# ckallidonis/mugiq

Hardware: AMD Instinct MI355X
Metric: loop_trace_sites_per_sec (higher is better)
Workload: dtype f64; 1 GPU; 32x32x32x32 fp64 N_ev=200 ultra-local 16-gamma loop (order FLOAT2); n_ev=200, partition=independent site blocks, one per rank

## Files before the change

### mugiq_amd/csrc/prolong.hip

```cpp
#include "mg_common.h"

#include <algorithm>
#include <vector>

namespace mugiq {

template <typename F, typename A> struct ProlongArgs {
  const Cplx<F> *V;
  int64_t Vpo;
  int Vstride;
  int NV;
  int X[4], Xc[4], bs[4];
  int spinBs;
  int volumeCB;
  const void *const *coarse;
  int64_t Cpo;
  int Cstride;
  const void *const *fine;
  int Fstride;
  int64_t Fpo;
  int nVec;
  const A *inv_sigma;
  Cplx<A> *loop;
};

template <typename F, typename A, int ORDER, bool WRITE, bool CONTRACT, bool STAGED>
__global__ __launch_bounds__(kPrTile *kPrGroups) void prolong_kernel(ProlongArgs<F, A> a) {
  extern __shared__ __align__(16) unsigned char smem[];
  Cplx<F> *Vt = reinterpret_cast<Cplx<F> *>(smem);
  const int tilesPerParity = (a.volumeCB + kPrTile - 1) / kPrTile;
  const int pty = blockIdx.x / tilesPerParity;
  const int x0 = (blockIdx.x - pty * tilesPerParity) * kPrTile;
  const int t = threadIdx.x, site = t & (kPrTile - 1), g = t / kPrTile;
  const int x_cb = x0 + site;
  const bool valid = x_cb < a.volumeCB;

  if constexpr (STAGED) {
    const int nPl = 12 * a.NV;
    for (int k = g; k < nPl; k += kPrGroups)
      Vt[k * kPrTile + site] = valid ? a.V[pty * a.Vpo + (int64_t)k * a.Vstride + x_cb] : Cplx<F>{F(0), F(0)};
    __syncthreads();
  }
  const Cplx<F> *Vg = a.V + pty * a.Vpo + (valid ? x_cb : a.volumeCB - 1);

  int c[4] = {0, 0, 0, 0};
  if (valid) get_coords(c, x_cb, a.X, pty);
  int cc[4];
#pragma unroll
  for (int d = 0; d < 4; d++) cc[d] = c[d] / a.bs[d];
  const int cpar = (cc[0] + cc[1] + cc[2] + cc[3]) & 1;
  const int64_t coff = (int64_t)cpar * a.Cpo + (lex_index(cc, a.Xc) >> 1);

  A diag[4] = {A(0), A(0), A(0), A(0)};
  Cplx<A> up[6];
#pragma unroll
  for (int i = 0; i < 6; i++) up[i] = Cplx<A>{A(0), A(0)};

  for (int nb = 0; nb < a.nVec; nb += 2 * kPrGroups) {
    const int n0 = nb + 2 * g, n1 = n0 + 1;
    if (n0 >= a.nVec) continue;
    const bool has1 = n1 < a.nVec;
    const Cplx<F> *c0 = static_cast<const Cplx<F> *>(a.coarse[n0]) + coff;
    const Cplx<F> *c1 = static_cast<const Cplx<F> *>(a.coarse[has1 ? n1 : n0]) + coff;
    Cplx<A> o0[12], o1[12];
#pragma unroll
    for (int k = 0; k < 12; k++) o0[k] = o1[k] = Cplx<A>{A(0), A(0)};
    typedef F vec2 __attribute__((ext_vector_type(2)));
    Cplx<F> sv0[12], sv1[12], sv2[12];
    vec2 sp0[4], sp1[4], sp2[4];
#define MUGIQ_PR_LOAD(sv, sp, jexpr)                                                                                   \
  {                                                                                                                    \
    const int j_ = (jexpr) < a.NV ? (jexpr) : a.NV - 1;                                                                \
    _Pragma("unroll") for (int chi = 0; chi < 2; chi++) {                                                              \
      sp[chi] = *as_global(reinterpret_cast<const vec2 *>(c0 + (int64_t)(chi * a.NV + j_) * a.Cstride));               \
      sp[2 + chi] = *as_global(reinterpret_cast<const vec2 *>(c1 + (int64_t)(chi * a.NV + j_) * a.Cstride));           \
    }                                                                                                                  \
    _Pragma("unroll") for (int sc = 0; sc < 12; sc++) {                                                                \
      if constexpr (STAGED) sv[sc] = Vt[(sc * a.NV + j_) * kPrTile + site];                                            \
      else sv[sc] = Vg[(int64_t)(sc * a.NV + j_) * a.Vstride];                                                         \
    }                                                                                                                  \
  }
#define MUGIQ_PR_COMPUTE(sv, sp)                                                                                       \
  {                                                                                                                    \
    const Cplx<A> p0[2] = {Cplx<A>{(A)sp[0].x, (A)sp[0].y}, Cplx<A>{(A)sp[1].x, (A)sp[1].y}};                          \
    const Cplx<A> p1[2] = {Cplx<A>{(A)sp[2].x, (A)sp[2].y}, Cplx<A>{(A)sp[3].x, (A)sp[3].y}};                          \
    _Pragma("unroll") for (int sc = 0; sc < 12; sc++) {                                                                \
      const Cplx<A> v{(A)sv[sc].re, (A)sv[sc].im};                                                                     \
      const int chi = (sc / 3) / 2;               \
      cmadd(o0[sc], v, p0[chi]);                                                                                       \
      cmadd(o1[sc], v, p1[chi]);                                                                                       \
    }                                                                                                                  \
  }
    if constexpr (CONTRACT) {
      for (int j = 0; j < a.NV; j++) {
        MUGIQ_PR_LOAD(sv0, sp0, j)
        MUGIQ_PR_COMPUTE(sv0, sp0)
      }
    } else {
      MUGIQ_PR_LOAD(sv0, sp0, 0)
      MUGIQ_PR_LOAD(sv1, sp1, 1)
      for (int j = 0; j < a.NV; j += 3) {
        MUGIQ_PR_LOAD(sv2, sp2, j + 2)
        MUGIQ_PR_COMPUTE(sv0, sp0)
        MUGIQ_PR_LOAD(sv0, sp0, j + 3)
        if (j + 1 < a.NV) MUGIQ_PR_COMPUTE(sv1, sp1)
        MUGIQ_PR_LOAD(sv1, sp1, j + 4)
        if (j + 2 < a.NV) MUGIQ_PR_COMPUTE(sv2, sp2)
      }
    }
#undef MUGIQ_PR_LOAD
#undef MUGIQ_PR_COMPUTE
    if constexpr (WRITE) {
      if (valid) {
        Cplx<F> w[12];
#pragma unroll
        for (int k = 0; k < 12; k++) w[k] = Cplx<F>{(F)o0[k].re, (F)o0[k].im};
        SpinorView<F, ORDER>{const_cast<F *>(static_cast<const F *>(a.fine[n0])), a.Fstride, a.Fpo}.store(w, pty, x_cb);
        if (has1) {
#pragma unroll
          for (int k = 0; k < 12; k++) w[k] = Cplx<F>{(F)o1[k].re, (F)o1[k].im};
          SpinorView<F, ORDER>{const_cast<F *>(static_cast<const F *>(a.fine[n1])), a.Fstride, a.Fpo}.store(w, pty, x_cb);
        }
      }
    }
    if constexpr (CONTRACT) {
      accumulate_herm(diag, up, o0, a.inv_sigma[n0]);
      if (has1) accumulate_herm(diag, up, o1, a.inv_sigma[n1]);
    }
  }

  if constexpr (CONTRACT) {
    __syncthreads();
    A *red = reinterpret_cast<A *>(smem);
#pragma unroll
    for (int i = 0; i < 4; i++) red[(i * kPrGroups + g) * kPrTile + site] = diag[i];
#pragma unroll
    for (int i = 0; i < 6; i++) {
      red[((4 + 2 * i) * kPrGroups + g) * kPrTile + site] = up[i].re;
      red[((5 + 2 * i) * kPrGroups + g) * kPrTile + site] = up[i].im;
    }
    __syncthreads();
    if (g == 0 && valid) {
      A sum[16];
#pragma unroll
      for (int i = 0; i < 16; i++) {
        A s = A(0);
        for (int gg = 0; gg < kPrGroups; gg++) s += red[(i * kPrGroups + gg) * kPrTile + site];
        sum[i] = s;
      }
      Cplx<A> acc[16];
      int p = 0;
#pragma unroll
      for (int be = 0; be < 4; be++) {
        acc[be * 4 + be] = Cplx<A>{sum[be], A(0)};
#pragma unroll
        for (int al = be + 1; al < 4; al++) {
          acc[be * 4 + al] = Cplx<A>{sum[4 + 2 * p], sum[5 + 2 * p]};
          acc[al * 4 + be] = Cplx<A>{sum[4 + 2 * p], -sum[5 + 2 * p]};
          p++;
        }
      }
      trace_and_store(a.loop, acc, 2 * a.volumeCB, x_cb + pty * a.volumeCB);
    }
  }
}

int validate_transfer(const MugiqHipTransfer *T, const MugiqHipCoarseField *c0, const char *who) {
  MUGIQ_REQUIRE(T && T->V, "%s: transfer / null vectors are NULL", who);
  MUGIQ_REQUIRE(T->precision == 4 || T->precision == 8, "%s: transfer precision %d", who, T->precision);
  MUGIQ_REQUIRE(T->nVec >= 1 && T->nVec <= 64, "%s: n_vec = %d must be in [1, 64]", who, T->nVec);
  MUGIQ_REQUIRE(T->spinBlockSize == 2, "%s: spin_block_size = %d (the reference's drivers use 2, tests/loop.cpp:569)", who, T->spinBlockSize);
  long long vol = 1, volc = 1;
  for (int d = 0; d < 4; d++) {
    MUGIQ_REQUIRE(T->X[d] > 0 && (T->X[d] & 1) == 0, "%s: fine X[%d] = %d must be positive and even", who, d, T->X[d]);
    MUGIQ_REQUIRE(T->geoBlockSize[d] >= 1 && T->X[d] % T->geoBlockSize[d] == 0, "%s: geo_block_size[%d] = %d does not divide X = %d", who, d, T->geoBlockSize[d], T->X[d]);
    const int xc = T->X[d] / T->geoBlockSize[d];
    MUGIQ_REQUIRE((xc & 1) == 0, "%s: coarse extent %d in dim %d must be even (even-odd coarse field)", who, xc, d);
    MUGIQ_REQUIRE(c0->X[d] == xc, "%s: coarse field X[%d] = %d, expected %d", who, d, c0->X[d], xc);
    vol *= T->X[d];
    volc *= xc;
  }
  MUGIQ_REQUIRE(T->stride >= vol / 2 && T->parity_offset >= (int64_t)12 * T->nVec * T->stride, "%s: V stride / parity_offset too small", who);
  MUGIQ_REQUIRE(c0->data && c0->precision == T->precision && c0->nSpin == 2 && c0->nColor == T->nVec, "%s: coarse field must have precision %d, nSpin 2, nColor %d", who, T->precision, T->nVec);
  MUGIQ_REQUIRE(c0->volumeCB == volc / 2 && c0->stride >= c0->volumeCB && c0->parity_offset >= (int64_t)2 * T->nVec * c0->stride, "%s: coarse field geometry mismatch", who);
  return MUGIQ_HIP_SUCCESS;
}

template <typename Args> static void set_lattices(Args &a, const TransferGeom &g) {
  for (int d = 0; d < 4; d++) a.X[d] = g.X[d], a.Xc[d] = g.Xc[d], a.bs[d] = g.bs[d];
}
template <typename Args> static void set_geometry(Args &a, const TransferGeom &g) {
  set_lattices(a, g);
  a.volumeCB = g.volumeCB, a.volumeCBc = g.volumeCBc, a.aggVol = g.aggVol;
}

template <typename F, typename A, int ORDER, bool WRITE, bool CONTRACT, typename Form>
static int launch_prolong(const Form &form, bool staged, const MugiqHipTransfer *T, const MugiqHipCoarseField *coarse, const MugiqHipSpinorField *fine,
                          const double *sigma, void *loop_d, int nVec, hipStream_t stream) {
  const size_t pb = sizeof(void *) * (size_t)nVec;
  std::vector<unsigned char> host(2 * pb + sizeof(A) * (size_t)nVec);
  const void **hc = reinterpret_cast<const void **>(host.data());
  const void **hf = reinterpret_cast<const void **>(host.data() + pb);
  A *hs = reinterpret_cast<A *>(host.data() + 2 * pb);
  for (int n = 0; n < nVec; n++) {
    hc[n] = coarse[n].data;
    hf[n] = WRITE ? fine[n].data : nullptr;
    hs[n] = CONTRACT ? static_cast<A>(1.0 / static_cast<F>(sigma[n])) : A(0);
  }
  void *dev = nullptr;
  int st = upload_table(&dev, host.data(), host.size(), stream);
  if (st) return st;
  ProlongArgs<F, A> a;
  a.V = static_cast<const Cplx<F> *>(T->V);
  a.Vpo = T->parity_offset;
  a.Vstride = T->stride;
  a.NV = T->nVec;
  set_lattices(a, form.geom);
  a.spinBs = T->spinBlockSize;
  a.volumeCB = form.geom.volumeCB;
  a.coarse = reinterpret_cast<const void *const *>(dev);
  a.Cpo = coarse[0].parity_offset;
  a.Cstride = coarse[0].stride;
  a.fine = reinterpret_cast<const void *const *>(static_cast<unsigned char *>(dev) + pb);
  a.Fstride = WRITE ? fine[0].stride : 0;
  a.Fpo = WRITE ? fine[0].parity_offset : 0;
  a.nVec = nVec;
  a.inv_sigma = reinterpret_cast<const A *>(static_cast<unsigned char *>(dev) + 2 * pb);
  a.loop = static_cast<Cplx<A> *>(loop_d);
  if constexpr (sizeof(F) == 8)
    if (!staged) return launch_with_lds(prolong_kernel<F, A, ORDER, WRITE, CONTRACT, false>, form.workgroups, form.threads, form.ldsBytes, stream, a);
  return launch_with_lds(prolong_kernel<F, A, ORDER, WRITE, CONTRACT, true>, form.workgroups, form.threads, form.ldsBytes, stream, a);
}


constexpr int kPcEvecs = 8;
template <typename F> struct ProlongCoarseArgs {
  const Cplx<F> *V;
  int64_t Vpo;
  int Vstride, NV, NCf;
  int X[4], Xc[4], bs[4];
  int volumeCB;
  const void *const *in;
  int64_t Ipo, Opo;
  int Istride, Ostride, nVec;
};

template <typename F> __global__ __launch_bounds__(128) void prolong_coarse_kernel(ProlongCoarseArgs<F> a) {
  const int tid = blockIdx.x * blockDim.x + threadIdx.x;
  if (tid >= 2 * a.volumeCB) return;
  const int pty = tid / a.volumeCB, x_cb = tid - pty * a.volumeCB;
  const int k = blockIdx.y, s = k / a.NCf;
  const int n0 = blockIdx.z * kPcEvecs;
  int c[4], cc[4];
  get_coords(c, x_cb, a.X, pty);
#pragma unroll
  for (int d = 0; d < 4; d++) cc[d] = c[d] / a.bs[d];
  const int cpar = (cc[0] + cc[1] + cc[2] + cc[3]) & 1;
  const int64_t coff = (int64_t)cpar * a.Ipo + (lex_index(cc, a.Xc) >> 1);
  const Cplx<F> *inp[kPcEvecs];
#pragma unroll
  for (int i = 0; i < kPcEvecs; i++) {
    const int n = n0 + i < a.nVec ? n0 + i : a.nVec - 1;
    inp[i] = static_cast<const Cplx<F> *>(as_constant(a.in)[n]) + coff + (int64_t)(s * a.NV) * a.Istride;
  }
  Cplx<F> acc[kPcEvecs];
#pragma unroll
  for (int i = 0; i < kPcEvecs; i++) acc[i] = Cplx<F>{F(0), F(0)};
  const Cplx<F> *vp = a.V + (int64_t)pty * a.Vpo + (int64_t)k * a.NV * a.Vstride + x_cb;
  for (int j = 0; j < a.NV; j++) {
    const Cplx<F> v = vp[(int64_t)j * a.Vstride];
#pragma unroll
    for (int i = 0; i < kPcEvecs; i++) {
      typedef F vec2 __attribute__((ext_vector_type(2)));
      const vec2 u = *as_global(reinterpret_cast<const vec2 *>(inp[i] + (int64_t)j * a.Istride));
      cmadd(acc[i], v, Cplx<F>{u.x, u.y});
    }
  }
#pragma unroll
  for (int i = 0; i < kPcEvecs; i++)
    if (n0 + i < a.nVec) {
      Cplx<F> *o = static_cast<Cplx<F> *>(const_cast<void *>(as_constant(a.in)[a.nVec + n0 + i]));
      o[(int64_t)pty * a.Opo + (int64_t)k * a.Ostride + x_cb] = acc[i];
    }
}

template <typename F>
static int launch_prolong_coarse(const MugiqHipCoarseField *out, const MugiqHipCoarseField *in, int nVec, const MugiqHipTransfer *T,
                                 hipStream_t stream) {
  std::vector<const void *> host(2 * (size_t)nVec);
  for (int n = 0; n < nVec; n++) {
    host[n] = in[n].data;
    host[nVec + n] = out[n].data;
  }
  void *dev = nullptr;
  int st = upload_table(&dev, host.data(), host.size() * sizeof(void *), stream);
  if (st) return st;
  ProlongCoarseArgs<F> a;
  a.V = static_cast<const Cplx<F> *>(T->V);
  a.Vpo = T->parity_offset;
  a.Vstride = T->stride;
  a.NV = T->nVec;
  a.NCf = out[0].nColor;
  set_lattices(a, transfer_geom(*T));
  a.volumeCB = out[0].volumeCB;
  a.in = reinterpret_cast<const void *const *>(dev);
  a.Ipo = in[0].parity_offset;
  a.Istride = in[0].stride;
  a.Opo = out[0].parity_offset;
  a.Ostride = out[0].stride;
  a.nVec = nVec;
  const dim3 grid((2 * a.volumeCB + 127) / 128, 2 * a.NCf, (nVec + kPcEvecs - 1) / kPcEvecs);
  hipLaunchKernelGGL((prolong_coarse_kernel<F>), grid, dim3(128), 0, stream, a);
  MUGIQ_CHECK_HIP(hipGetLastError());
  return MUGIQ_HIP_SUCCESS;
}

template <typename F, typename A> struct CoarseOuterArgs {
  const void *const *coarse;
  const A *inv_sigma;
  int nVec, NV, volumeCBc, Cstride;
  int64_t Cpo;
  Cplx<A> *C;
};

constexpr int kCoEvecs = 8;
constexpr int kCoMaxNC = 64;

template <typename F, typename A, int B> __global__ __launch_bounds__(256) void coarse_outer_kernel(CoarseOuterArgs<F, A> a) {
  __shared__ Cplx<A> ph[kCoEvecs][kCoMaxNC], phs[kCoEvecs][kCoMaxNC];
  const int NC = 2 * a.NV;
  const int site = xcd_contiguous_block(blockIdx.x, gridDim.x);
  const int pty = site / a.volumeCBc, x_cb = site - pty * a.volumeCBc;
  const int r0 = (threadIdx.x >> 4) * B, c0 = (threadIdx.x & 15) * B;
  Cplx<A> acc[B][B];
#pragma unroll
  for (int i = 0; i < B; i++)
#pragma unroll
    for (int j = 0; j < B; j++) acc[i][j] = Cplx<A>{A(0), A(0)};
  for (int n0 = 0; n0 < a.nVec; n0 += kCoEvecs) {
    __syncthreads();
    for (int idx = threadIdx.x; idx < kCoEvecs * kCoMaxNC; idx += 256) {
      const int nn = idx / kCoMaxNC, comp = idx - nn * kCoMaxNC, n = n0 + nn;
      Cplx<A> v{A(0), A(0)}, vs{A(0), A(0)};
      if (n < a.nVec && comp < NC) {
        typedef F vec2 __attribute__((ext_vector_type(2)));
        const Cplx<F> *c = static_cast<const Cplx<F> *>(as_constant(a.coarse)[n]) + (int64_t)pty * a.Cpo + (int64_t)comp * a.Cstride + x_cb;
        const vec2 u = *as_global(reinterpret_cast<const vec2 *>(c));
        const A s = as_constant(a.inv_sigma)[n];
        v = Cplx<A>{(A)u.x, (A)u.y};
        vs = Cplx<A>{s * v.re, s * v.im};
      }
      ph[nn][comp] = v;
      phs[nn][comp] = vs;
    }
    __syncthreads();
#pragma unroll
    for (int nn = 0; nn < kCoEvecs; nn++) {
      Cplx<A> x[B], y[B];
#pragma unroll
      for (int i = 0; i < B; i++) {
        x[i] = phs[nn][(r0 + i) & (kCoMaxNC - 1)];
        y[i] = ph[nn][(c0 + i) & (kCoMaxNC - 1)];
      }
#pragma unroll
      for (int i = 0; i < B; i++)
#pragma unroll
        for (int j = 0; j < B; j++) {
          acc[i][j].re = fma(x[i].re, y[j].re, acc[i][j].re);
          acc[i][j].re = fma(x[i].im, y[j].im, acc[i][j].re);
          acc[i][j].im = fma(x[i].im, y[j].re, acc[i][j].im);
          acc[i][j].im = fma(-x[i].re, y[j].im, acc[i][j].im);
        }
    }
  }
  Cplx<A> *out = a.C + (int64_t)site * NC * NC;
#pragma unroll
  for (int i = 0; i < B; i++)
#pragma unroll
    for (int j = 0; j < B; j++)
      if (r0 + i < NC && c0 + j < NC) out[(r0 + i) * NC + c0 + j] = acc[i][j];
}


template <typename F, typename A> struct FineCongruenceArgs {
  const Cplx<F> *V;
  int64_t Vpo;
  int Vstride, NV;
  int X[4], Xc[4], bs[4];
  int volumeCB, volumeCBc, aggVol;
  const Cplx<A> *C;
  Cplx<A> *loop;
};

template <typename F, typename A, int JC, int SPR, int NH>
__global__ __launch_bounds__(4 * NH * SPR) void fine_congruence_kernel(FineCongruenceArgs<F, A> a) {
  extern __shared__ __align__(16) unsigned char smem[];
  const int NV = a.NV, NC = 2 * NV;
  Cplx<A> *Cs = reinterpret_cast<Cplx<A> *>(smem);
  Cplx<A> *red = Cs + NC * NC;
  Cplx<F> *Vs = reinterpret_cast<Cplx<F> *>(red + SPR * 16);
  constexpr int LPS = 4 * NH, NT = LPS * SPR;
  const int t = threadIdx.x, sidx = t / LPS, lane = t % LPS, hh = lane >> 2, q = lane & 3, chi = q >> 1, chip = q & 1;

  int cc[4], r = xcd_contiguous_block(blockIdx.x, gridDim.x);
#pragma unroll
  for (int d = 0; d < 4; d++) {
    cc[d] = r % a.Xc[d];
    r /= a.Xc[d];
  }
  const int cpar = (cc[0] + cc[1] + cc[2] + cc[3]) & 1;
  const Cplx<A> *Cg = a.C + ((int64_t)cpar * a.volumeCBc + (lex_index(cc, a.Xc) >> 1)) * (int64_t)(NC * NC);
  for (int i = t; i < NC * NC; i += NT) Cs[i] = Cg[i];

  auto member = [&](int k, int &pty, int &x_cb) { aggregate_member(a.bs, a.X, cc, min(k, a.aggVol - 1), &pty, &x_cb); };

  const int rounds = (a.aggVol + SPR - 1) / SPR;
  const int stSite = t % SPR, stRow0 = t / SPR;
  for (int rd = 0; rd < rounds; rd++) {
    int myP, myX, stP, stX;
    member(rd * SPR + sidx, myP, myX);
    member(rd * SPR + stSite, stP, stX);
    Cplx<A> blk[2][2];
#pragma unroll
    for (int i = 0; i < 2; i++) blk[i][0] = blk[i][1] = Cplx<A>{A(0), A(0)};
    for (int c = 0; c < 3; c++) {
      __syncthreads();
      for (int row = stRow0; row < 4 * NV; row += LPS) {
        const int sp = row / NV, j = row - sp * NV;
        typedef F vec2 __attribute__((ext_vector_type(2)));
        const Cplx<F> *src = a.V + (int64_t)stP * a.Vpo + (int64_t)((3 * sp + c) * NV + j) * a.Vstride + stX;
        const vec2 u = *as_global(reinterpret_cast<const vec2 *>(src));
        Vs[row * SPR + stSite] = Cplx<F>{u.x, u.y};
      }
      __syncthreads();
      const Cplx<F> *u0p = Vs + (2 * chi) * NV * SPR + sidx, *u1p = u0p + NV * SPR;
      const Cplx<F> *w0p = Vs + (2 * chip) * NV * SPR + sidx, *w1p = w0p + NV * SPR;
      {
        const int h = hh * JC;
        Cplx<A> T0[JC], T1[JC];
#pragma unroll
        for (int jj = 0; jj < JC; jj++) T0[jj] = T1[jj] = Cplx<A>{A(0), A(0)};
        const Cplx<A> *crow = Cs + (chi * NV) * NC + chip * NV + h;
        for (int j = 0; j < NV; j++) {
          const Cplx<F> a0 = u0p[j * SPR], a1 = u1p[j * SPR];
          const Cplx<A> u0{(A)a0.re, (A)a0.im}, u1{(A)a1.re, (A)a1.im};
#pragma unroll
          for (int jj = 0; jj < JC; jj++) {
            const Cplx<A> cv = crow[j * NC + jj];
            cmadd(T0[jj], u0, cv);
            cmadd(T1[jj], u1, cv);
          }
        }
#pragma unroll
        for (int jj = 0; jj < JC; jj++) {
          const Cplx<F> b0 = w0p[(h + jj) * SPR], b1 = w1p[(h + jj) * SPR];
          const Cplx<A> w0{(A)b0.re, (A)b0.im}, w1{(A)b1.re, (A)b1.im};
          cmadd_conj(blk[0][0], w0, T0[jj]);
          cmadd_conj(blk[0][1], w1, T0[jj]);
          cmadd_conj(blk[1][0], w0, T1[jj]);
          cmadd_conj(blk[1][1], w1, T1[jj]);
        }
      }
    }
#pragma unroll
    for (int m = 4; m < LPS; m <<= 1)
#pragma unroll
      for (int b2 = 0; b2 < 2; b2++)
#pragma unroll
        for (int a2 = 0; a2 < 2; a2++) {
          blk[b2][a2].re += __shfl_xor(blk[b2][a2].re, m);
          blk[b2][a2].im += __shfl_xor(blk[b2][a2].im, m);
        }
    if (hh == 0) {
#pragma unroll
      for (int b2 = 0; b2 < 2; b2++)
#pragma unroll
        for (int a2 = 0; a2 < 2; a2++) red[sidx * 16 + (2 * chip + a2) * 4 + (2 * chi + b2)] = blk[b2][a2];
    }
    __syncthreads();
    if (hh == 0 && rd * SPR + sidx < a.aggVol) {
      Cplx<A> full[16];
#pragma unroll
      for (int i = 0; i < 16; i++) full[i] = red[sidx * 16 + i];
      const int site = myX + myP * a.volumeCB;
      if (q == 0) trace_and_store_range<A, 0, 4>(a.loop, full, 2 * a.volumeCB, site);
      else if (q == 1) trace_and_store_range<A, 4, 8>(a.loop, full, 2 * a.volumeCB, site);
      else if (q == 2) trace_and_store_range<A, 8, 12>(a.loop, full, 2 * a.volumeCB, site);
      else trace_and_store_range<A, 12, 16>(a.loop, full, 2 * a.volumeCB, site);
    }
  }
}

template <typename F> struct CongruenceMfmaArgs {
  const Cplx<F> *V;
  int64_t Vpo;
  int Vstride;
  int X[4], Xc[4], bs[4];
  int volumeCB, volumeCBc, aggVol;
  const Cplx<double> *C;
  Cplx<double> *loop;
};

template <typename F, int NV, bool GLDS> __global__ __launch_bounds__(64 * (NV / 2)) void fine_congruence_mfma_kernel(CongruenceMfmaArgs<F> a) {
  typedef double d4 __attribute__((ext_vector_type(4)));
  typedef F vec2 __attribute__((ext_vector_type(2)));
  constexpr int NC = 2 * NV, KS = NV / 2, NCB = NV / 4, NW = 2 * NCB, NT = 64 * NW;
  constexpr int ROWS = 12 * NV;
  constexpr int LDV = kCmS;
  constexpr int NLD = (ROWS * kCmS) / NT;
  extern __shared__ __align__(16) unsigned char smem[];
  Cplx<double> *Vs0 = reinterpret_cast<Cplx<double> *>(smem);
  double *red = reinterpret_cast<double *>(Vs0 + (GLDS ? 2 : 1) * ROWS * LDV);
  const int t = threadIdx.x, lane = t & 63, wave = __builtin_amdgcn_readfirstlane(t >> 6);
  const int chi = wave / NCB, cb = wave - chi * NCB;
  const int chip = cb / (NCB / 2), jb = (cb - chip * (NCB / 2)) * 8;
  const int kq = lane >> 4, site = lane & 15;

  int cc[4], rr = xcd_contiguous_block(blockIdx.x, gridDim.x);
#pragma unroll
  for (int d = 0; d < 4; d++) {
    cc[d] = rr % a.Xc[d];
    rr /= a.Xc[d];
  }
  const int cpar = (cc[0] + cc[1] + cc[2] + cc[3]) & 1;
  const Cplx<double> *Cg = a.C + ((int64_t)cpar * a.volumeCBc + (lex_index(cc, a.Xc) >> 1)) * (int64_t)(NC * NC);
  double cfrag[KS];
#pragma unroll
  for (int m = 0; m < KS / 2; m++) {
    const Cplx<double> cv = Cg[(chi * NV + 4 * m + kq) * NC + 8 * cb + (site >> 1)];
    cfrag[2 * m] = (site & 1) == 0 ? cv.re : cv.im;
    cfrag[2 * m + 1] = (site & 1) == 0 ? -cv.im : cv.re;
  }
  auto member = [&](int k, int &pty, int &x_cb) { aggregate_member(a.bs, a.X, cc, k, &pty, &x_cb); };
  vec2 u[GLDS ? 1 : NLD];
  const int stSite = t & 15;
  auto fetch = [&](int rd, Cplx<double> *buf) {
    int pty, x_cb;
    member(rd * kCmS + stSite, pty, x_cb);
    const Cplx<F> *base = a.V + (int64_t)pty * a.Vpo + x_cb;
#pragma unroll
    for (int q = 0; q < NLD; q++) {
      const int row = (t + NT * q) >> 4;
      if constexpr (GLDS) {
#if defined(__HIP_DEVICE_COMPILE__)
        typedef __attribute__((address_space(3))) void lds_void;
        __builtin_amdgcn_global_load_lds(as_global(reinterpret_cast<const vec2 *>(base + (int64_t)row * a.Vstride)),
                                         (lds_void *)(buf + (wave * 64 + NT * q)), 16, 0, 0);
#endif
      } else {
        u[q] = *as_global(reinterpret_cast<const vec2 *>(base + (int64_t)row * a.Vstride));
      }
    }
  };
  auto commit = [&](Cplx<double> *buf) {
    if constexpr (!GLDS) {
#pragma unroll
      for (int q = 0; q < NLD; q++) buf[t + NT * q] = Cplx<double>{(double)u[q].x, (double)u[q].y};
    }
  };
  const int bBase = kq * LDV + site, wBase = (jb + (kq >> 1)) * LDV + site;
  const int rT = kq & 1;

  const int rounds = a.aggVol / kCmS;
  fetch(0, Vs0);
  for (int rd = 0; rd < rounds; rd++) {
    Cplx<double> *Vs = Vs0 + (GLDS ? (rd & 1) * ROWS * LDV : 0);
    if constexpr (GLDS) {
      asm volatile("s_waitcnt vmcnt(0)" ::: "memory");
      __syncthreads();
      if (rd + 1 < rounds) fetch(rd + 1, Vs0 + ((rd + 1) & 1) * ROWS * LDV);
    } else {
      __syncthreads();
      commit(Vs);
      if (rd + 1 < rounds) fetch(rd + 1, Vs);
      __syncthreads();
    }
    double blk[2][2][2];
#pragma unroll
    for (int i = 0; i < 8; i++) (&blk[0][0][0])[i] = 0.0;
    Cplx<double> bfA[KS / 2], bfB[KS / 2], w[2][4];
#define MUGIQ_CM_LOAD_B(bf_, u_)                                                                          \
  {                                                                                                       \
    const int rowB_ = ((2 * chi + ((u_) & 1)) * 3 + ((u_) >> 1)) * NV;                                    \
    _Pragma("unroll") for (int m = 0; m < KS / 2; m++) bf_[m] = Vs[(rowB_ + 4 * m) * LDV + bBase];        \
  }
#define MUGIQ_CM_UNIT(bf_, bfNext_, u_)                                                                   \
  {                                                                                                       \
    if ((u_) + 1 < 6) MUGIQ_CM_LOAD_B(bfNext_, (u_) + 1)                                                  \
    if (((u_) & 1) == 0) {                                                                                \
      _Pragma("unroll") for (int ai = 0; ai < 2; ai++)                                                    \
        _Pragma("unroll") for (int r = 0; r < 4; r++)                                                     \
          w[ai][r] = Vs[(((2 * chip + ai) * 3 + ((u_) >> 1)) * NV + 2 * r) * LDV + wBase];                \
    }                                                                                                     \
    __builtin_amdgcn_sched_barrier(0);  \
    d4 acc = {0, 0, 0, 0};                                                                                \
    _Pragma("unroll") for (int m = 0; m < KS / 2; m++) {                                                  \
      acc = __builtin_amdgcn_mfma_f64_16x16x4f64(cfrag[2 * m], bf_[m].re, acc, 0, 0, 0);                  \
      acc = __builtin_amdgcn_mfma_f64_16x16x4f64(cfrag[2 * m + 1], bf_[m].im, acc, 0, 0, 0);              \
    }                                                                                                     \
                          \
    _Pragma("unroll") for (int ai = 0; ai < 2; ai++)                                                      \
      _Pragma("unroll") for (int r = 0; r < 4; r++) {                                                     \
        const double wa = rT == 0 ? w[ai][r].re : w[ai][r].im;                \
        const double wb = rT == 0 ? -w[ai][r].im : w[ai][r].re;               \
        blk[(u_) & 1][ai][0] = fma(acc[r], wa, blk[(u_) & 1][ai][0]);                                     \
        blk[(u_) & 1][ai][1] = fma(acc[r], wb, blk[(u_) & 1][ai][1]);                                     \
      }                                                                                                   \
  }
    MUGIQ_CM_LOAD_B(bfA, 0)
    MUGIQ_CM_UNIT(bfA, bfB, 0)
    MUGIQ_CM_UNIT(bfB, bfA, 1)
    MUGIQ_CM_UNIT(bfA, bfB, 2)
    MUGIQ_CM_UNIT(bfB, bfA, 3)
    MUGIQ_CM_UNIT(bfA, bfB, 4)
    MUGIQ_CM_UNIT(bfB, bfA, 5)
#undef MUGIQ_CM_UNIT
#undef MUGIQ_CM_LOAD_B
#pragma unroll
    for (int i = 0; i < 8; i++) {
      double v = (&blk[0][0][0])[i];
      v += __shfl_xor(v, 16);
      v += __shfl_xor(v, 32);
      (&blk[0][0][0])[i] = v;
    }
    if (kq == 0) {
#pragma unroll
      for (int i = 0; i < 8; i++) red[(wave * kCmS + site) * 8 + i] = (&blk[0][0][0])[i];
    }
    asm volatile("s_waitcnt lgkmcnt(0)" ::: "memory");
    __builtin_amdgcn_s_barrier();
    asm volatile("" ::: "memory");
    if (t < 4 * kCmS) {
      const int s = t >> 2, q = t & 3;
      Cplx<double> full[16];
#pragma unroll
      for (int al = 0; al < 4; al++)
#pragma unroll
        for (int be = 0; be < 4; be++) {
          const int w0 = (be >> 1) * NCB + (al >> 1) * (NCB / 2);
          double re = 0.0, im = 0.0;
#pragma unroll
          for (int wv = 0; wv < NCB / 2; wv++) {
            const double *p = red + ((w0 + wv) * kCmS + s) * 8 + ((be & 1) * 2 + (al & 1)) * 2;
            re += p[0];
            im += p[1];
          }
          full[al * 4 + be] = Cplx<double>{re, im};
        }
      Cplx<double> tr[4];
      if (q == 0) traces_range<double, 0>(tr, full);
      else if (q == 1) traces_range<double, 4>(tr, full);
      else if (q == 2) traces_range<double, 8>(tr, full);
      else traces_range<double, 12>(tr, full);
      int pty, x_cb;
      member(rd * kCmS + s, pty, x_cb);
      double *out = reinterpret_cast<double *>(a.loop + (int64_t)(2 * a.volumeCB) * (4 * q) + x_cb + pty * a.volumeCB);
#pragma unroll
      for (int i = 0; i < 4; i++) {
        unsafeAtomicAdd(out + (int64_t)(4 * a.volumeCB) * i, tr[i].re);
        unsafeAtomicAdd(out + (int64_t)(4 * a.volumeCB) * i + 1, tr[i].im);
      }
    }
  }
}

template <typename F, int NV> static int launch_congruence_mfma(const ContractForm &form, const CongruenceMfmaArgs<F> &a, hipStream_t stream) {
  return launch_with_lds(fine_congruence_mfma_kernel<F, NV, congruence_mfma_glds(sizeof(F), NV)>, form.workgroups, form.threads, form.ldsBytes, stream, a);
}

template <typename F, typename A>
static int coarse_plan(const ContractForm &form, const MugiqHipTransfer *T, const MugiqHipCoarseField *coarse, const double *sigma, void *loop_d,
                       int nVec, hipStream_t stream) {
  const int NV = T->nVec;
  const TransferGeom &g = form.geom;
  const size_t pb = sizeof(void *) * (size_t)nVec;
  void *base = nullptr;
  int st = stream_scratch(&base, form.scratchBytes, stream);
  if (st) return st;
  std::vector<unsigned char> host(form.tableBytes, 0);
  const void **hc = reinterpret_cast<const void **>(host.data());
  A *hs = reinterpret_cast<A *>(host.data() + pb);
  for (int n = 0; n < nVec; n++) {
    hc[n] = coarse[n].data;
    hs[n] = static_cast<A>(1.0 / static_cast<F>(sigma[n]));
  }
  void *dev = nullptr;
  if ((st = upload_table(&dev, host.data(), form.tableBytes, stream))) return st;
  MUGIQ_REQUIRE(dev == base, "prolongateContract: scratch moved under the coarse-grid plan");
  CoarseOuterArgs<F, A> o;
  o.coarse = reinterpret_cast<const void *const *>(dev);
  o.inv_sigma = reinterpret_cast<const A *>(static_cast<unsigned char *>(dev) + pb);
  o.nVec = nVec;
  o.NV = NV;
  o.volumeCBc = g.volumeCBc;
  o.Cstride = coarse[0].stride;
  o.Cpo = coarse[0].parity_offset;
  o.C = reinterpret_cast<Cplx<A> *>(static_cast<unsigned char *>(dev) + form.tableBytes);
  const dim3 sites((unsigned)form.workgroups);
  switch (form.outerB) {
  case 1: hipLaunchKernelGGL((coarse_outer_kernel<F, A, 1>), sites, dim3(256), 0, stream, o); break;
  case 2: hipLaunchKernelGGL((coarse_outer_kernel<F, A, 2>), sites, dim3(256), 0, stream, o); break;
  case 3: hipLaunchKernelGGL((coarse_outer_kernel<F, A, 3>), sites, dim3(256), 0, stream, o); break;
  default: hipLaunchKernelGGL((coarse_outer_kernel<F, A, 4>), sites, dim3(256), 0, stream, o); break;
  }
  MUGIQ_CHECK_HIP(hipGetLastError());

  if constexpr (sizeof(A) == 8) {
    if (form.family == MUGIQ_HIP_CONTRACT_FAMILY_COARSE_MFMA) {
      CongruenceMfmaArgs<F> m;
      m.V = static_cast<const Cplx<F> *>(T->V);
      m.Vpo = T->parity_offset;
      m.Vstride = T->stride;
      set_geometry(m, g);
      m.C = reinterpret_cast<const Cplx<double> *>(o.C);
      m.loop = static_cast<Cplx<double> *>(loop_d);
      switch (NV) {
      case 8: return launch_congruence_mfma<F, 8>(form, m, stream);
      case 16: return launch_congruence_mfma<F, 16>(form, m, stream);
      case 24: return launch_congruence_mfma<F, 24>(form, m, stream);
      default: return launch_congruence_mfma<F, 32>(form, m, stream);
      }
    }
  }
  FineCongruenceArgs<F, A> a;
  a.V = static_cast<const Cplx<F> *>(T->V);
  a.Vpo = T->parity_offset;
  a.Vstride = T->stride;
  a.NV = NV;
  set_geometry(a, g);
  a.C = o.C;
  a.loop = static_cast<Cplx<A> *>(loop_d);
  switch (100 * form.JC + form.SPR + form.NH) {
#define MUGIQ_CONGRUENCE_CASE(J, S, H) \
  case 100 * J + S + H: return launch_with_lds(fine_congruence_kernel<F, A, J, S, H>, form.workgroups, form.threads, form.ldsBytes, stream, a);
    MUGIQ_CONGRUENCE_CASE(12, 64, 2) MUGIQ_CONGRUENCE_CASE(12, 32, 2) MUGIQ_CONGRUENCE_CASE(12, 64, 1) MUGIQ_CONGRUENCE_CASE(12, 32, 1)
    MUGIQ_CONGRUENCE_CASE(8, 64, 1) MUGIQ_CONGRUENCE_CASE(8, 32, 1) MUGIQ_CONGRUENCE_CASE(8, 64, 2) MUGIQ_CONGRUENCE_CASE(8, 32, 2)
    MUGIQ_CONGRUENCE_CASE(8, 64, 4) MUGIQ_CONGRUENCE_CASE(8, 32, 4)
#undef MUGIQ_CONGRUENCE_CASE
  }
  return set_error(MUGIQ_HIP_ERROR_UNSUPPORTED, "prolongateContract: no congruence kernel with %d columns, %d sites, %d chunks", form.JC, form.SPR, form.NH);
}



struct ProlongMfmaArgs {
  const Cplx<double> *V;
  int64_t Vpo;
  int Vstride;
  int X[4], Xc[4], bs[4];
  int volumeCB, volumeCBc, aggVol;
  const void *const *table;
  const Cplx<double> *packed;
  int64_t Cpo;
  int Cstride;
  int Fstride;
  int64_t Fpo;
  int nVec, nVec8;
  int blkBegin, blkCount;
};

__global__ __launch_bounds__(256) void coarse_pack_kernel(ProlongMfmaArgs a, int NV) {
  __shared__ Cplx<double> tile[16][17];
  const int nT = (a.nVec8 + 15) / 16;
  const int xt = blockIdx.x, cj = blockIdx.y, nt = blockIdx.z % nT, cpar = blockIdx.z / nT;
  const int hi = threadIdx.x >> 4, lo = threadIdx.x & 15;
  {
    const int n = nt * 16 + hi, xc = xt * 16 + lo;
    Cplx<double> v{0.0, 0.0};
    if (n < a.nVec && xc < a.volumeCBc) v = static_cast<const Cplx<double> *>(a.table[n])[(int64_t)cpar * a.Cpo + (int64_t)cj * a.Cstride + xc];
    tile[hi][lo] = v;
  }
  __syncthreads();
  const int xc = xt * 16 + hi, n = nt * 16 + lo;
  if (xc < a.volumeCBc && n < a.nVec8)
    const_cast<Cplx<double> *>(a.packed)[(((int64_t)cpar * a.volumeCBc + xc) * (2 * NV) + cj) * a.nVec8 + n] = tile[lo][hi];
}

template <int NV> __global__ __launch_bounds__(64 * kPmWaves) void prolong_mfma_kernel(ProlongMfmaArgs a) {
  typedef double d4 __attribute__((ext_vector_type(4)));
  typedef double vec2 __attribute__((ext_vector_type(2)));
  constexpr int KS = NV / 2;
  constexpr int ROWS = 12 * NV, LDV = kCmS, NT = 64 * kPmWaves, NLD = (ROWS * kCmS) / NT;
  static_assert((ROWS * kCmS) % NT == 0 && NV % 8 == 0, "tile staging assumes whole wave instructions");
  extern __shared__ __align__(16) unsigned char smem[];
  Cplx<double> *Vs0 = reinterpret_cast<Cplx<double> *>(smem);
  const int t = threadIdx.x, lane = t & 63, wave = __builtin_amdgcn_readfirstlane(t >> 6);
  const int kq = lane >> 4, site = lane & 15;
  const int chi = wave & 1, b0 = wave >> 1;
  int npairs = 0;
#pragma unroll
  for (int i = 0; i < kPmPairs; i++)
    if (b0 + 4 * i < a.blkCount) npairs = i + 1;

  int cc[4], rr = xcd_contiguous_block(blockIdx.x, gridDim.x);
#pragma unroll
  for (int d = 0; d < 4; d++) {
    cc[d] = rr % a.Xc[d];
    rr /= a.Xc[d];
  }
  const int cpar = (cc[0] + cc[1] + cc[2] + cc[3]) & 1;

  double afrag[kPmPairs][KS];
  Cplx<double> *fineP[kPmPairs][2];
  {
    const int rowA = lane & 15, riA = (rowA >> 2) & 1;
    const Cplx<double> *pk = a.packed + (((int64_t)cpar * a.volumeCBc + (lex_index(cc, a.Xc) >> 1)) * 2 + chi) * (int64_t)NV * a.nVec8 +
                             (int64_t)kq * a.nVec8 + (rowA & 3) + 4 * (rowA >> 3);
#pragma unroll
    for (int i = 0; i < kPmPairs; i++) {
      const int b = a.blkBegin + (npairs > 0 ? b0 + (i < npairs ? 4 * i : 0) : 0);
#pragma unroll
      for (int m = 0; m < KS / 2; m++) {
        const vec2 cv = *as_global(reinterpret_cast<const vec2 *>(pk + (int64_t)(4 * m) * a.nVec8 + 8 * b));
        afrag[i][2 * m] = riA == 0 ? cv.x : cv.y;
        afrag[i][2 * m + 1] = riA == 0 ? -cv.y : cv.x;
      }
#pragma unroll
      for (int h = 0; h < 2; h++) {
        const int ns = 8 * b + kq + 4 * h;
        fineP[i][h] = ns < a.nVec ? static_cast<Cplx<double> *>(const_cast<void *>(a.table[a.nVec + ns])) : nullptr;
      }
    }
  }
  auto member = [&](int k, int &pty, int &x_cb) { aggregate_member(a.bs, a.X, cc, k, &pty, &x_cb); };
  const int stSite = t & 15;
  auto fetch = [&](int rd, Cplx<double> *buf) {
    int pty, x_cb;
    member(rd * kCmS + stSite, pty, x_cb);
    const Cplx<double> *base = a.V + (int64_t)pty * a.Vpo + x_cb;
#pragma unroll
    for (int q = 0; q < NLD; q++) {
      const int row = (t + NT * q) >> 4;
      (void)row, (void)base, (void)buf;
#if defined(__HIP_DEVICE_COMPILE__)
      typedef __attribute__((address_space(3))) void lds_void;
      __builtin_amdgcn_global_load_lds(as_global(reinterpret_cast<const vec2 *>(base + (int64_t)row * a.Vstride)),
                                       (lds_void *)(buf + (wave * 64 + NT * q)), 16, 0, 0);
#endif
    }
  };

  const int rounds = a.aggVol / kCmS;
  fetch(0, Vs0);
  for (int rd = 0; rd < rounds; rd++) {
    const Cplx<double> *Vs = Vs0 + (rd & 1) * ROWS * LDV;
    asm volatile("s_waitcnt vmcnt(0)" ::: "memory");
    __syncthreads();
    if (rd + 1 < rounds) fetch(rd + 1, Vs0 + ((rd + 1) & 1) * ROWS * LDV);
    int pty, x_cb;
    member(rd * kCmS + site, pty, x_cb);
    const int64_t foff = (int64_t)pty * a.Fpo + x_cb;
#pragma unroll 1
    for (int scl = 0; scl < 6; scl++) {
      const int sc = 6 * chi + scl;
      Cplx<double> bf[KS / 2];
#pragma unroll
      for (int m = 0; m < KS / 2; m++) bf[m] = Vs[(sc * NV + 4 * m + kq) * LDV + site];
      const int64_t soff = foff + (int64_t)sc * a.Fstride;
#define MUGIQ_PM_STORE(i_, acc_)                                                                                        \
  {                                                                                                                     \
    if (fineP[i_][0]) *as_global(reinterpret_cast<vec2 *>(fineP[i_][0] + soff)) = vec2{acc_[0], acc_[1]};               \
    if (fineP[i_][1]) *as_global(reinterpret_cast<vec2 *>(fineP[i_][1] + soff)) = vec2{acc_[2], acc_[3]};               \
  }
#pragma unroll
      for (int i = 0; i < kPmPairs; i += 2) {
        if (i + 1 < npairs) {
          const int i1 = i + 1 < kPmPairs ? i + 1 : i;
          d4 acc0 = {0, 0, 0, 0}, acc1 = {0, 0, 0, 0};
#pragma unroll
          for (int m = 0; m < KS / 2; m++) {
            acc0 = __builtin_amdgcn_mfma_f64_16x16x4f64(afrag[i][2 * m], bf[m].re, acc0, 0, 0, 0);
            acc1 = __builtin_amdgcn_mfma_f64_16x16x4f64(afrag[i1][2 * m], bf[m].re, acc1, 0, 0, 0);
            acc0 = __builtin_amdgcn_mfma_f64_16x16x4f64(afrag[i][2 * m + 1], bf[m].im, acc0, 0, 0, 0);
            acc1 = __builtin_amdgcn_mfma_f64_16x16x4f64(afrag[i1][2 * m + 1], bf[m].im, acc1, 0, 0, 0);
          }
          MUGIQ_PM_STORE(i, acc0)
          MUGIQ_PM_STORE(i1, acc1)
        } else if (i < npairs) {
          d4 acc0 = {0, 0, 0, 0};
#pragma unroll
          for (int m = 0; m < KS / 2; m++) {
            acc0 = __builtin_amdgcn_mfma_f64_16x16x4f64(afrag[i][2 * m], bf[m].re, acc0, 0, 0, 0);
            acc0 = __builtin_amdgcn_mfma_f64_16x16x4f64(afrag[i][2 * m + 1], bf[m].im, acc0, 0, 0, 0);
          }
          MUGIQ_PM_STORE(i, acc0)
        }
      }
#undef MUGIQ_PM_STORE
    }
  }
}

static int launch_prolong_mfma(const ProlongForm &form, const MugiqHipTransfer *T, const MugiqHipCoarseField *coarse, const MugiqHipSpinorField *fine,
                               int nVec, void *packed_ws, hipStream_t stream) {
  const int NV = T->nVec;
  ProlongMfmaArgs a;
  a.V = static_cast<const Cplx<double> *>(T->V);
  a.Vpo = T->parity_offset;
  a.Vstride = T->stride;
  set_geometry(a, form.geom);
  a.Cpo = coarse[0].parity_offset;
  a.Cstride = coarse[0].stride;
  a.Fstride = fine[0].stride;
  a.Fpo = fine[0].parity_offset;
  a.nVec = nVec;
  a.nVec8 = (nVec + 7) / 8 * 8;
  std::vector<const void *> host(2 * (size_t)nVec);
  for (int n = 0; n < nVec; n++) {
    host[n] = coarse[n].data;
    host[nVec + n] = fine[n].data;
  }
  void *dev = nullptr;
  int st = upload_table(&dev, host.data(), sizeof(void *) * host.size(), stream);
  if (st) return st;
  a.table = reinterpret_cast<const void *const *>(dev);
  a.packed = static_cast<const Cplx<double> *>(packed_ws);
  const int nVec16 = (a.nVec8 + 15) / 16;
  hipLaunchKernelGGL(coarse_pack_kernel, dim3((unsigned)((a.volumeCBc + 15) / 16), (unsigned)(2 * NV), (unsigned)(2 * nVec16)), dim3(256), 0, stream, a, NV);
  MUGIQ_CHECK_HIP(hipGetLastError());
  const int blocks = a.nVec8 / 8;
  for (int b = 0; b < blocks; b += form.blocksPerPass) {
    a.blkBegin = b;
    a.blkCount = std::min(form.blocksPerPass, blocks - b);
    void (*kern)(ProlongMfmaArgs) = prolong_mfma_kernel<8>;
    if (NV == 16) kern = prolong_mfma_kernel<16>;
    else if (NV == 24) kern = prolong_mfma_kernel<24>;
    if ((st = launch_with_lds(kern, form.workgroups, form.threads, form.ldsBytes, stream, a))) return st;
  }
  return MUGIQ_HIP_SUCCESS;
}

int validate_coarse_transfer(const MugiqHipTransfer *T, const MugiqHipCoarseField *out_h, const MugiqHipCoarseField *in_h, int nVec, const char *who) {
  MUGIQ_REQUIRE(out_h && in_h && nVec >= 1, "%s: NULL / empty argument", who);
  MUGIQ_REQUIRE(T && T->V, "%s: Transfer operator for this level does not exist!", who);
  MUGIQ_REQUIRE(T->precision == 4 || T->precision == 8, "%s: transfer precision %d", who, T->precision);
  MUGIQ_REQUIRE(T->nVec >= 1 && T->nVec <= 96, "%s: n_vec = %d must be in [1, 96]", who, T->nVec);
  MUGIQ_REQUIRE(T->spinBlockSize == 1, "%s: spin_block_size = %d: a coarse level keeps both chiralities (1)", who, T->spinBlockSize);
  const MugiqHipCoarseField &o = out_h[0], &i = in_h[0];
  MUGIQ_REQUIRE(o.nSpin == 2 && i.nSpin == 2 && i.nColor == T->nVec && o.nColor >= 1 && o.nColor <= 96, "%s: fields must have nSpin 2; coarser nColor = n_vec = %d", who, T->nVec);
  long long vol = 1, volc = 1;
  for (int d = 0; d < 4; d++) {
    MUGIQ_REQUIRE(T->X[d] > 0 && (T->X[d] & 1) == 0 && o.X[d] == T->X[d], "%s: finer lattice X[%d] = %d (field: %d) must be positive, even and equal", who, d, T->X[d], o.X[d]);
    MUGIQ_REQUIRE(T->geoBlockSize[d] >= 1 && T->X[d] % T->geoBlockSize[d] == 0, "%s: geo_block_size[%d] = %d does not divide X = %d", who, d, T->geoBlockSize[d], T->X[d]);
    const int xc = T->X[d] / T->geoBlockSize[d];
    MUGIQ_REQUIRE((xc & 1) == 0 && i.X[d] == xc, "%s: coarser extent in dim %d must be even and equal X/block = %d (field: %d)", who, d, xc, i.X[d]);
    vol *= T->X[d];
    volc *= xc;
  }
  MUGIQ_REQUIRE(o.volumeCB == vol / 2 && i.volumeCB == volc / 2, "%s: volumeCB mismatch", who);
  MUGIQ_REQUIRE(T->stride >= vol / 2 && T->parity_offset >= (int64_t)2 * o.nColor * T->nVec * T->stride, "%s: V stride / parity_offset too small", who);
  for (int n = 0; n < nVec; n++) {
    MUGIQ_REQUIRE(out_h[n].data && in_h[n].data && out_h[n].data != in_h[n].data, "%s: field %d is NULL or aliased", who, n);
    MUGIQ_REQUIRE(out_h[n].precision == T->precision && in_h[n].precision == T->precision, "%s: field %d: precision differs from the transfer's", who, n);
    MUGIQ_REQUIRE(out_h[n].stride == o.stride && out_h[n].parity_offset == o.parity_offset && out_h[n].nColor == o.nColor &&
                      in_h[n].stride == i.stride && in_h[n].parity_offset == i.parity_offset && in_h[n].nColor == i.nColor,
                  "%s: field %d differs in layout from field 0", who, n);
  }
  MUGIQ_REQUIRE(o.stride >= o.volumeCB && o.parity_offset >= (int64_t)2 * o.nColor * o.stride && i.stride >= i.volumeCB &&
                    i.parity_offset >= (int64_t)2 * i.nColor * i.stride, "%s: field stride / parity_offset too small", who);
  return MUGIQ_HIP_SUCCESS;
}

int prolong_batched(const MugiqHipSpinorField *fine, const MugiqHipCoarseField *coarse, int nVec, const MugiqHipTransfer *T, const TransferSwitches &sw,
                    void *packed_ws, hipStream_t s) {
  const ProlongForm form = select_prolong_form(*T, T->precision, fine[0].field_order, nVec, sw);
  if (form.family == MUGIQ_HIP_PROLONG_FAMILY_MFMA) return launch_prolong_mfma(form, T, coarse, fine, nVec, packed_ws, s);
  const bool staged = form.family == MUGIQ_HIP_PROLONG_FAMILY_VECTOR_STAGED;
  switch (10 * form.precision + form.order) {
  case 82: return launch_prolong<double, double, 2, true, false>(form, staged, T, coarse, fine, nullptr, nullptr, nVec, s);
  case 84: return launch_prolong<double, double, 4, true, false>(form, staged, T, coarse, fine, nullptr, nullptr, nVec, s);
  case 42: return launch_prolong<float, float, 2, true, false>(form, staged, T, coarse, fine, nullptr, nullptr, nVec, s);
  default: return launch_prolong<float, float, 4, true, false>(form, staged, T, coarse, fine, nullptr, nullptr, nVec, s);
  }
}

int prolong_coarse_batched(const MugiqHipCoarseField *out, const MugiqHipCoarseField *in, int nVec, const MugiqHipTransfer *T, hipStream_t s) {
  if (T->precision == 8) return launch_prolong_coarse<double>(out, in, nVec, T, s);
  return launch_prolong_coarse<float>(out, in, nVec, T, s);
}

}

using namespace mugiq;

extern "C" {

int mugiq_hip_prolongate_batched(const MugiqHipSpinorField *fine_h, const MugiqHipCoarseField *coarse_h, int nVec,
                                 const MugiqHipTransfer *transfer, void *stream) {
  if (int dbg_ = mugiq::debug_poison_lds_if_asked(static_cast<hipStream_t>(stream))) return dbg_;
  const char *who = "prolongateEvec";
  MUGIQ_REQUIRE(fine_h && coarse_h && nVec >= 1, "%s: NULL / empty argument", who);
  int st = validate_transfer(transfer, &coarse_h[0], who);
  if (st) return st;
  for (int n = 0; n < nVec; n++) {
    if ((st = validate_spinor(&fine_h[n], who, "fineEvec"))) return st;
    MUGIQ_REQUIRE(same_geometry(fine_h[n], fine_h[0]), "%s: fine field %d differs in geometry from field 0", who, n);
    MUGIQ_REQUIRE(coarse_h[n].data && coarse_h[n].stride == coarse_h[0].stride && coarse_h[n].parity_offset == coarse_h[0].parity_offset &&
                      coarse_h[n].precision == coarse_h[0].precision, "%s: coarse field %d differs from field 0", who, n);
  }
  MUGIQ_REQUIRE(fine_h[0].precision == transfer->precision, "%s: fine precision %d != transfer precision %d", who, fine_h[0].precision, transfer->precision);
  for (int d = 0; d < 4; d++) MUGIQ_REQUIRE(fine_h[0].X[d] == transfer->X[d], "%s: fine X[%d] mismatch", who, d);
  hipStream_t s = static_cast<hipStream_t>(stream);
  const TransferSwitches sw = transfer_switches_from_env();
  const ProlongForm form = select_prolong_form(*transfer, transfer->precision, fine_h[0].field_order, nVec, sw);
  void *packed = nullptr;
  if (form.family == MUGIQ_HIP_PROLONG_FAMILY_MFMA && (st = stream_workspace(&packed, form.workspaceBytes, s))) return st;
  return prolong_batched(fine_h, coarse_h, nVec, transfer, sw, packed, s);
}

int mugiq_hip_prolongate_coarse_batched(const MugiqHipCoarseField *out_h, const MugiqHipCoarseField *in_h, int nVec,
                                        const MugiqHipTransfer *T, void *stream) {
// ... 40 lines not shown
```

Before: 156.5 million sites/s.

## Exploit Hermitian symmetry of coarse congruence to skip redundant MFMA spin blocks

```diff
diff --git a/mugiq_amd/csrc/prolong.hip b/mugiq_amd/csrc/prolong.hip
--- a/mugiq_amd/csrc/prolong.hip
+++ b/mugiq_amd/csrc/prolong.hip
@@ -1,6 +1,7 @@
 #include "mg_common.h"
 
 #include <algorithm>
+#include <type_traits>
 #include <vector>
 
 namespace mugiq {
@@ -321,6 +322,7 @@
   int nVec, NV, volumeCBc, Cstride;
   int64_t Cpo;
   Cplx<A> *C;
+  static constexpr bool kHermitian = std::is_floating_point<A>::value;
 };
 
 constexpr int kCoEvecs = 8;
@@ -489,6 +491,13 @@
       else trace_and_store_range<A, 12, 16>(a.loop, full, 2 * a.volumeCB, site);
     }
   }
+}
+
+constexpr unsigned long long pack_gamma_rows(const int (&table)[16][4], int half) {
+  unsigned long long v = 0;
+  for (int g = 0; g < 8; g++)
+    for (int s2 = 0; s2 < 4; s2++) v |= (unsigned long long)table[8 * half + g][s2] << (2 * (4 * g + s2));
+  return v;
 }
 
 template <typename F> struct CongruenceMfmaArgs {
@@ -515,6 +524,10 @@
   const int chi = wave / NCB, cb = wave - chi * NCB;
   const int chip = cb / (NCB / 2), jb = (cb - chip * (NCB / 2)) * 8;
   const int kq = lane >> 4, site = lane & 15;
+  constexpr bool SPLIT = NCB / 2 == 3;
+  constexpr int KW = SPLIT ? 3 * KS / 4 : KS, KH = KS - KW;
+  const bool mirror = chi == 1 && chip == 0;
+  const int hchi = cb >> 1, hchip = (cb + 1) >> 1;
 
   int cc[4], rr = xcd_contiguous_block(blockIdx.x, gridDim.x);
 #pragma unroll
@@ -524,12 +537,20 @@
   }
   const int cpar = (cc[0] + cc[1] + cc[2] + cc[3]) & 1;
   const Cplx<double> *Cg = a.C + ((int64_t)cpar * a.volumeCBc + (lex_index(cc, a.Xc) >> 1)) * (int64_t)(NC * NC);
+  auto cval = [&](int chi_, int cb_, int k) {
+    const Cplx<double> cv = Cg[(chi_ * NV + 4 * (k >> 1) + kq) * NC + 8 * cb_ + (site >> 1)];
+    if ((k & 1) == 0) return (site & 1) == 0 ? cv.re : cv.im;
+    return (site & 1) == 0 ? -cv.im : cv.re;
+  };
   double cfrag[KS];
-#pragma unroll
-  for (int m = 0; m < KS / 2; m++) {
-    const Cplx<double> cv = Cg[(chi * NV + 4 * m + kq) * NC + 8 * cb + (site >> 1)];
-    cfrag[2 * m] = (site & 1) == 0 ? cv.re : cv.im;
-    cfrag[2 * m + 1] = (site & 1) == 0 ? -cv.im : cv.re;
+  if (SPLIT && mirror) {
+#pragma unroll
+    for (int lb = 0; lb < 3; lb++)
+#pragma unroll
+      for (int kk = 0; kk < KH; kk++) cfrag[lb * KH + kk] = cval(hchi, hchip * (NCB / 2) + lb, KW + kk);
+  } else {
+#pragma unroll
+    for (int k = 0; k < KW; k++) cfrag[k] = cval(chi, cb, k);
   }
   auto member = [&](int k, int &pty, int &x_cb) { aggregate_member(a.bs, a.X, cc, k, &pty, &x_cb); };
   vec2 u[GLDS ? 1 : NLD];
@@ -578,11 +599,12 @@
     double blk[2][2][2];
 #pragma unroll
     for (int i = 0; i < 8; i++) (&blk[0][0][0])[i] = 0.0;
-    Cplx<double> bfA[KS / 2], bfB[KS / 2], w[2][4];
+    if (!mirror) {
+    Cplx<double> bfA[(KW + 1) / 2], bfB[(KW + 1) / 2], w[2][4];
 #define MUGIQ_CM_LOAD_B(bf_, u_)                                                                          \
   {                                                                                                       \
     const int rowB_ = ((2 * chi + ((u_) & 1)) * 3 + ((u_) >> 1)) * NV;                                    \
-    _Pragma("unroll") for (int m = 0; m < KS / 2; m++) bf_[m] = Vs[(rowB_ + 4 * m) * LDV + bBase];        \
+    _Pragma("unroll") for (int m = 0; m < (KW + 1) / 2; m++) bf_[m] = Vs[(rowB_ + 4 * m) * LDV + bBase];  \
   }
 #define MUGIQ_CM_UNIT(bf_, bfNext_, u_)                                                                   \
   {                                                                                                       \
@@ -594,10 +616,8 @@
     }                                                                                                     \
     __builtin_amdgcn_sched_barrier(0);  \
     d4 acc = {0, 0, 0, 0};                                                                                \
-    _Pragma("unroll") for (int m = 0; m < KS / 2; m++) {                                                  \
-      acc = __builtin_amdgcn_mfma_f64_16x16x4f64(cfrag[2 * m], bf_[m].re, acc, 0, 0, 0);                  \
-      acc = __builtin_amdgcn_mfma_f64_16x16x4f64(cfrag[2 * m + 1], bf_[m].im, acc, 0, 0, 0);              \
-    }                                                                                                     \
+    _Pragma("unroll") for (int k = 0; k < KW; k++)                                                        \
+      acc = __builtin_amdgcn_mfma_f64_16x16x4f64(cfrag[k], (k & 1) ? bf_[k >> 1].im : bf_[k >> 1].re, acc, 0, 0, 0); \
                           \
     _Pragma("unroll") for (int ai = 0; ai < 2; ai++)                                                      \
       _Pragma("unroll") for (int r = 0; r < 4; r++) {                                                     \
@@ -616,50 +636,105 @@
     MUGIQ_CM_UNIT(bfB, bfA, 5)
 #undef MUGIQ_CM_UNIT
 #undef MUGIQ_CM_LOAD_B
-#pragma unroll
-    for (int i = 0; i < 8; i++) {
-      double v = (&blk[0][0][0])[i];
-      v += __shfl_xor(v, 16);
-      v += __shfl_xor(v, 32);
-      (&blk[0][0][0])[i] = v;
-    }
-    if (kq == 0) {
-#pragma unroll
-      for (int i = 0; i < 8; i++) red[(wave * kCmS + site) * 8 + i] = (&blk[0][0][0])[i];
+    } else if constexpr (SPLIT) {
+      const int wBaseH = (kq >> 1) * LDV + site;
+#pragma unroll
+      for (int c = 0; c < 3; c++) {
+        double hb[2][KH];
+        Cplx<double> w[2][4];
+#pragma unroll
+        for (int b2 = 0; b2 < 2; b2++)
+#pragma unroll
+          for (int kk = 0; kk < KH; kk++) {
+            const Cplx<double> &v = Vs[(((2 * hchi + b2) * 3 + c) * NV + 4 * ((KW + kk) >> 1)) * LDV + bBase];
+            hb[b2][kk] = ((KW + kk) & 1) ? v.im : v.re;
+          }
+#pragma unroll
+        for (int ai = 0; ai < 2; ai++)
+#pragma unroll
+          for (int r = 0; r < 4; r++) w[ai][r] = Vs[(((2 * hchip + ai) * 3 + c) * NV + 2 * r) * LDV + wBaseH];
+        __builtin_amdgcn_sched_barrier(0);
+        d4 acc[2][3];
+#pragma unroll
+        for (int i = 0; i < 6; i++) (&acc[0][0])[i] = d4{0, 0, 0, 0};
+#pragma unroll
+        for (int kk = 0; kk < KH; kk++)
+#pragma unroll
+          for (int b2 = 0; b2 < 2; b2++)
+#pragma unroll
+            for (int lb = 0; lb < 3; lb++) acc[b2][lb] = __builtin_amdgcn_mfma_f64_16x16x4f64(cfrag[lb * KH + kk], hb[b2][kk], acc[b2][lb], 0, 0, 0);
+#pragma unroll
+        for (int lb = 0; lb < 3; lb++) {
+          if (lb > 0) {
+#pragma unroll
+            for (int ai = 0; ai < 2; ai++)
+#pragma unroll
+              for (int r = 0; r < 4; r++) w[ai][r] = Vs[(((2 * hchip + ai) * 3 + c) * NV + 8 * lb + 2 * r) * LDV + wBaseH];
+          }
+#pragma unroll
+          for (int b2 = 0; b2 < 2; b2++)
+#pragma unroll
+            for (int ai = 0; ai < 2; ai++)
+#pragma unroll
+              for (int r = 0; r < 4; r++) {
+                const double wa = rT == 0 ? w[ai][r].re : w[ai][r].im;
+                const double wb = rT == 0 ? -w[ai][r].im : w[ai][r].re;
+                blk[b2][ai][0] = fma(acc[b2][lb][r], wa, blk[b2][ai][0]);
+                blk[b2][ai][1] = fma(acc[b2][lb][r], wb, blk[b2][ai][1]);
+              }
+        }
+      }
+    }
+    if (SPLIT || !mirror) {
+#pragma unroll
+      for (int i = 0; i < 8; i++) {
+        double v = (&blk[0][0][0])[i];
+        v += __shfl_xor(v, 16);
+        v += __shfl_xor(v, 32);
+        (&blk[0][0][0])[i] = v;
+      }
+      if (kq == 0) {
+#pragma unroll
+        for (int i = 0; i < 8; i++) red[(wave * kCmS + site) * 8 + i] = (&blk[0][0][0])[i];
+      }
     }
     asm volatile("s_waitcnt lgkmcnt(0)" ::: "memory");
     __builtin_amdgcn_s_barrier();
     asm volatile("" ::: "memory");
-    if (t < 4 * kCmS) {
-      const int s = t >> 2, q = t & 3;
-      Cplx<double> full[16];
-#pragma unroll
-      for (int al = 0; al < 4; al++)
-#pragma unroll
-        for (int be = 0; be < 4; be++) {
-          const int w0 = (be >> 1) * NCB + (al >> 1) * (NCB / 2);
-          double re = 0.0, im = 0.0;
-#pragma unroll
-          for (int wv = 0; wv < NCB / 2; wv++) {
-            const double *p = red + ((w0 + wv) * kCmS + s) * 8 + ((be & 1) * 2 + (al & 1)) * 2;
-            re += p[0];
-            im += p[1];
-          }
-          full[al * 4 + be] = Cplx<double>{re, im};
+    if (t < 16 * kCmS) {
+      const int s = t & 15, g = t >> 4;
+      constexpr unsigned long long ph0 = pack_gamma_rows(kGammaPhase, 0), ph1 = pack_gamma_rows(kGammaPhase, 1);
+      constexpr unsigned long long col0 = pack_gamma_rows(kGammaColumn, 0), col1 = pack_gamma_rows(kGammaColumn, 1);
+      const unsigned long long phases = g < 8 ? ph0 : ph1, columns = g < 8 ? col0 : col1;
+      double tre = 0.0, tim = 0.0;
+#pragma unroll
+      for (int al = 0; al < 4; al++) {
+        const int sh = 2 * (4 * (g & 7) + al);
+        const int ph = (int)(phases >> sh) & 3, be = (int)(columns >> sh) & 3;
+        const bool derived = (be >> 1) > (al >> 1);
+        const int bb = derived ? al : be, aa = derived ? be : al;
+        const double *p = red + (((bb >> 1) * NCB + (aa >> 1) * (NCB / 2)) * kCmS + s) * 8 + ((bb & 1) * 2 + (aa & 1)) * 2;
+        double re = 0.0, im = 0.0;
+#pragma unroll
+        for (int wv = 0; wv < NCB / 2; wv++) {
+          re += p[wv * kCmS * 8];
+          im += p[wv * kCmS * 8 + 1];
         }
-      Cplx<double> tr[4];
-      if (q == 0) traces_range<double, 0>(tr, full);
-      else if (q == 1) traces_range<double, 4>(tr, full);
-      else if (q == 2) traces_range<double, 8>(tr, full);
-      else traces_range<double, 12>(tr, full);
+        if constexpr (SPLIT) {
+          const double *ph_ = red + ((NCB + (bb >> 1) + (aa >> 1)) * kCmS + s) * 8 + ((bb & 1) * 2 + (aa & 1)) * 2;
+          re += ph_[0];
+          im += ph_[1];
+        }
+        if (derived) im = -im;
+        const double x = (ph & 1) ? -im : re, y = (ph & 1) ? re : im;
+        tre += (ph & 2) ? -x : x;
+        tim += (ph & 2) ? -y : y;
+      }
       int pty, x_cb;
       member(rd * kCmS + s, pty, x_cb);
-      double *out = reinterpret_cast<double *>(a.loop + (int64_t)(2 * a.volumeCB) * (4 * q) + x_cb + pty * a.volumeCB);
-#pragma unroll
-      for (int i = 0; i < 4; i++) {
-        unsafeAtomicAdd(out + (int64_t)(4 * a.volumeCB) * i, tr[i].re);
-        unsafeAtomicAdd(out + (int64_t)(4 * a.volumeCB) * i + 1, tr[i].im);
-      }
+      double *out = reinterpret_cast<double *>(a.loop + (int64_t)(2 * a.volumeCB) * g + x_cb + pty * a.volumeCB);
+      unsafeAtomicAdd(out, tre);
+      unsafeAtomicAdd(out + 1, tim);
     }
   }
 }
@@ -707,6 +782,7 @@
 
   if constexpr (sizeof(A) == 8) {
     if (form.family == MUGIQ_HIP_CONTRACT_FAMILY_COARSE_MFMA) {
+      static_assert(CoarseOuterArgs<F, A>::kHermitian, "the matrix-pipe congruence needs one coarse set and real weights");
       CongruenceMfmaArgs<F> m;
       m.V = static_cast<const Cplx<F> *>(T->V);
       m.Vpo = T->parity_offset;
```

Result: no change. 156.5 million sites/s (median of 6 runs) (+0.0%).
